# Gaukler/PlainRenderer

Hardware: AMD Instinct MI355X
Metric: frames/sec full GI+shade+post @4K; %HBM roofline; 1/2/4/8-GPU scaling (higher is better)
Workload: dtype f32

## Files before the change

### plainrenderer_amd/csrc/kernels_fast/shading_fast.hip

```cpp
#include "../backend.h"
#include "../device/shading_common.h"
#include "../device/fastmath.h"
#include "../device/buffer_fetch.h"
#include "upscale_quad.h"
#include "pcf_taps.h"
#include <type_traits>
#include <map>

namespace plr {

namespace fastshade {

#ifndef PLR_SHADE_WAVES
#define PLR_SHADE_WAVES 5
#endif

PLR_DI float rcpf(float x) { return __builtin_amdgcn_rcpf(x); }
PLR_DI float rsqf(float x) { return __builtin_amdgcn_rsqf(x); }
PLR_DI float sqrtv(float x) { return __builtin_amdgcn_sqrtf(x); }
PLR_DI float fmin1(float a, float b) { return __builtin_fminf(a, b); }
PLR_DI float fmax1(float a, float b) { return __builtin_fmaxf(a, b); }
PLR_DI float fclamp(float x, float lo, float hi) { return __builtin_fminf(__builtin_fmaxf(x, lo), hi); }
PLR_DI float fmix(float a, float b, float t) { return a + (b - a) * t; }
PLR_DI float log2h(float x) { return __builtin_amdgcn_logf(x); }
PLR_DI float exp2h(float x) { return __builtin_amdgcn_exp2f(x); }
PLR_DI vec3 nrm(vec3 v) { return v * rsqf(dot(v, v)); }
PLR_DI float pow5(float x) { x = fmax1(x, 0.f); const float x2 = x * x; return x2 * x2 * x; }
PLR_DI float fpow(float x, float y) { return x <= 0.f ? 0.f : exp2h(y * log2h(x)); }

PLR_DI float rcpRN(float d) { const float r = rcpf(d); return __builtin_fmaf(__builtin_fmaf(-d, r, 1.f), r, r); }
PLR_DI float divRNr(float n, float d, float r) { const float q = n * r; return __builtin_fmaf(__builtin_fmaf(-d, q, n), r, q); }
PLR_DI float divRN(float n, float d) { return divRNr(n, d, rcpf(d)); }
PLR_DI float sqrtRN(float x) { const float r = rsqf(x), s = x * r; return __builtin_fmaf(__builtin_fmaf(-s, s, x), 0.5f * r, s); }

struct ViewRay { vec3 Vn; float su, sv; };
PLR_DI ViewRay exactViewRay(const GlobalUbo* __restrict__ g, int px, int py) {
#pragma clang fp contract(off)
    ViewRay o;
// ... 91 lines not shown
    linearCoord(u * (float)im.w, &i0, &a);
    linearCoord(v * (float)im.h, &j0, &b);
    int xb; float a2;
    edgePair(i0, a, im.w, &xb, &a2);
    const int y0 = clampi(j0, im.h), y1 = clampi(j0 + 1, im.h);
    const BufferDesc texels = texelBuffer(im.ptr, 8u);
    const uint4 q0 = fetch128(texels, __umul24((uint32_t)y0, (uint32_t)im.w) + (uint32_t)xb), q1 = fetch128(texels, __umul24((uint32_t)y1, (uint32_t)im.w) + (uint32_t)xb);
    const float a0 = 1.f - a2, b0 = 1.f - b;
    vec4 r(0.f);
    r = accumulateTexel(r, q0.x, q0.y, a0 * b0);
    r = accumulateTexel(r, q0.z, q0.w, a2 * b0);
    r = accumulateTexel(r, q1.x, q1.y, a0 * b);
    r = accumulateTexel(r, q1.z, q1.w, a2 * b);
    return r;
}

struct ShadeParams {
    ImgView color, depth, normal, albedo, specular, brdfLut, shadowMaps[4], ysh, cocg, volumetricLut, skyLut;
    const LightBuffer* light;
    const ShadowCascadeInfo* shadowInfo;
    const VolumetricLightingSettings* vol;
    const GlobalUbo* g;
    const ImgView* bindless;
    uint32_t bindlessCount;
    uint32_t cascadeCount;
    int coverW, coverH, yBase;
    int xBase;
    uint32_t* sig;
    ImgView noiseTex;
    const float4* pcfTaps;
    const float4* pcfTapsByPosition;
    uint32_t pcfPositions;
    const uint2* lutEnergyFootprint;
};

#define PLR_SHADE_UNIFORM_PARAMS const GlobalUbo* __restrict__ gUniform, const LightBuffer* __restrict__ lightUniform, const ShadowCascadeInfo* __restrict__ shadowUniform, \
                                 const VolumetricLightingSettings* __restrict__ volUniform
#define PLR_SHADE_ADOPT_UNIFORMS(P) do { (P).g = gUniform; (P).light = lightUniform; (P).shadowInfo = shadowUniform; (P).vol = volUniform; } while (0)
#define PLR_SHADE_UNIFORM_ARGS(P) (P).g, (P).light, (P).shadowInfo, (P).vol

struct PcfTapRow { float4 q[kPcfTaps / 2]; };
PLR_DI float calcShadow(vec3 pos, const ImgView& shadowMap, const float* __restrict__ m, float lssX, float lssY, const PcfTapRow& taps) {
    float cxy0, cxy1;
    uint32_t depthThreshold;
    {
#pragma clang fp contract(off)
        const float x = ((m[0] * pos.x + m[4] * pos.y) + m[8] * pos.z) + m[12];
        const float y = ((m[1] * pos.x + m[5] * pos.y) + m[9] * pos.z) + m[13];
        const float z = ((m[2] * pos.x + m[6] * pos.y) + m[10] * pos.z) + m[14];
        const float w = ((m[3] * pos.x + m[7] * pos.y) + m[11] * pos.z) + m[15];
        const float rw = rcpf(w);
        cxy0 = divRNr(x, w, rw) * 0.5f + 0.5f;
        cxy1 = divRNr(y, w, rw) * 0.5f + 0.5f;
        const float actualDepth = fclamp(divRNr(z, w, rw), 0.f, 1.f);
        const uint32_t t0 = (uint32_t)(actualDepth * 65535.f);
        const float r16 = 1.f / 65535.f;
        const float q1 = divRNr((float)(t0 + 1u), 65535.f, r16), q0 = divRNr((float)t0, 65535.f, r16);
        depthThreshold = q1 <= actualDepth ? t0 + 1u : (q0 <= actualDepth ? t0 : t0 - 1u);
    }
    const int w = shadowMap.w, h = shadowMap.h;
    const float fw = (float)w, fh = (float)h;
    const float bxw = fastm::clampCoord(cxy0 * fw), byh = fastm::clampCoord(cxy1 * fh);
    const float sxw = 0.03f * lssX * fw, syh = 0.03f * lssY * fh;
    const __amdgpu_buffer_rsrc_t map = __builtin_amdgcn_make_buffer_rsrc(shadowMap.ptr, 0, w * h * 2, 0x00020000);
    uint32_t lit = 0u;
    auto tap = [&](float ox, float oy) {
        const int xi = floorToInt(__builtin_fmaf(ox, sxw, bxw)), yi = floorToInt(__builtin_fmaf(oy, syh, byh));
// ... 39 lines not shown
        const float unscaled = (1.f - energyIncoming) * (1.f - energyOutgoing) * rcpf(3.1415f * (1.f - energyAverage));
        const vec3 den = 1.f - fresnelAverage * (1.f - energyAverage);
        const vec3 scaling = (fresnelAverage * fresnelAverage * energyAverage) * vec3(rcpf(den.x), rcpf(den.y), rcpf(den.z));
        return unscaled * scaling;
    } else if (MULTISCATTER == 1) {
        const float lobe = (1.f - energyOutgoing) * (1.f / PLR_GLSL_PI);
        const vec3 den = 1.f - fresnelAverage * (1.f - energyOutgoing);
        return (fresnelAverage * fresnelAverage * (energyOutgoing * lobe)) * vec3(rcpf(den.x), rcpf(den.y), rcpf(den.z));
    } else if (MULTISCATTER == 2) {
        return f0 * (rcpf(energyOutgoing) - 1.f) * singleScatteringLobe;
    }
    return vec3(0.f);
}

struct PixelInputs {
    float depth;
    uint32_t albedo, specular;
    uint32_t normal, normalH, normalV;
    uint2 ysh;
    uint32_t cocg;
};
PLR_DI vec3 decodeNormal(uint32_t texel) {
    const vec3 raw = fastm::unorm8x4(texel).xyz() * 2.f - 1.f;
    return raw * rsqf(fmax1(dot(raw, raw), 1e-30f));
}

struct SurfaceTerms {
    vec3 N, V, f0, diffuseColor, diffuseBRDFIntegral;
    float r, NoV, energyOutgoing;
    vec3 brdfLut;
};
struct DirectOut { vec3 direct; float pixelDepth; vec2 noiseTexel; };
template <int DIFFUSE_BRDF, int MULTISCATTER, bool GEOMETRIC_AA>
PLR_DI DirectOut shadeDirect(const ShadeParams& P, int px, int py, const ViewRay& vr, const PixelInputs& in, vec3 lightColor, SurfaceTerms* st, uint32_t* sigWord) {
    const GlobalUbo* g = P.g;
    const Surface surf = exactSurface(g, vr.Vn, in.depth);
    const vec3 passPos = surf.passPos;
    const float pixelDepth = surf.pixelDepth;

    const vec3 albedoTexel = fastm::unorm8x4(in.albedo).xyz();
    const vec3 specularTexel = fastm::unorm8x4(in.specular).xyz();
    const float metalic = specularTexel.z;
    float r = specularTexel.y;
    r = fmax1(r * r, 0.0045f);
    const vec3 albedo(sRGBToLinear1(albedoTexel.x), sRGBToLinear1(albedoTexel.y), sRGBToLinear1(albedoTexel.z));
    const vec3 diffuseColor = (1.f - metalic) * albedo;
    const vec3 N = decodeNormal(in.normal);
    const vec3 L = nrm(ld3(g->sunDirection));
    const vec3 V = vr.Vn;
    const vec3 H = nrm(V + L);
    if (GEOMETRIC_AA) {
        const vec3 N_U = decodeNormal(in.normalH) - N, N_V = decodeNormal(in.normalV) - N;
        const float variance = 0.25f * (dot(N_V, N_V) + dot(N_U, N_U));
        const float kernelRoughness2 = fmin1(2.f * variance, 0.18f);
        r = fclamp(sqrtv(r * r + kernelRoughness2), 0.f, 1.f);
    }
    const float NoH = fmax1(dot(N, H), 0.f);
    const float NdotL = dot(N, L);
    const float NoL = fclamp(NdotL, 0.f, 1.f);
    const float VoH = fabsf(dot(V, H));
    const float LoV = fmax1(dot(L, V), 0.f);
    const float NoV = fmax1(fabsf(dot(N, V)), 0.0001f);
    const vec3 f0 = vmix(vec3(0.04f), albedo, metalic);

    const ImgView noiseTex = P.noiseTex;
    const uint32_t noiseIndex = fastm::texelIndex((uint32_t)fastm::repeatIndex(px, noiseTex.w), (uint32_t)fastm::repeatIndex(py, noiseTex.h), (uint32_t)noiseTex.w);
    const uint32_t noiseWord = fetch16(texelBuffer(noiseTex.ptr, 2u), noiseIndex);
    const vec2 noiseTexel = fastm::unorm8x2(noiseWord);
    const uint32_t noiseByte = noiseWord & 0xffu;

    int cascadeIndex = 0;
#pragma unroll
    for (int cascade = 0; cascade < 3; cascade++) cascadeIndex += (cascade < (int)P.cascadeCount - 1 && pixelDepth >= P.shadowInfo->splits[cascade]) ? 1 : 0;
    PcfTapRow tapRow;
    {
        const bool byPosition = P.pcfTapsByPosition != nullptr;
        const uint8_t* base = byPosition ? (const uint8_t*)P.pcfTapsByPosition : (const uint8_t*)P.pcfTaps;
        const uint32_t rowStride = byPosition ? P.pcfPositions * 16u : 16u;
        const uint32_t laneOffset = byPosition ? noiseIndex * 16u : noiseByte * (uint32_t)(kPcfTaps / 2 * 16);
        const __amdgpu_buffer_rsrc_t table = __builtin_amdgcn_make_buffer_rsrc((void*)base, 0, 0x7fffffff, 0x00020000);
#pragma unroll
        for (int k = 0; k < kPcfTaps / 2; k++) {
            const auto q = __builtin_amdgcn_raw_buffer_load_b128(table, (int)laneOffset, (int)((uint32_t)k * rowStride), 0);
            __builtin_memcpy(&tapRow.q[k], &q, 16);
        }
    }
    float sunShadow = 0.f;
    for (bool pending = true; pending;) {
        int c = __builtin_amdgcn_readfirstlane(cascadeIndex);
        const bool mine = cascadeIndex == c;
        asm volatile("" : "+s"(c));
        if (mine) {
            const ImgView& m0 = P.shadowMaps[0];
            ImgView shadowMap;
            shadowMap.ptr = c == 0 ? m0.ptr : c == 1 ? P.shadowMaps[1].ptr : c == 2 ? P.shadowMaps[2].ptr : P.shadowMaps[3].ptr;
            shadowMap.w = c == 0 ? m0.w : c == 1 ? P.shadowMaps[1].w : c == 2 ? P.shadowMaps[2].w : P.shadowMaps[3].w;
            shadowMap.h = c == 0 ? m0.h : c == 1 ? P.shadowMaps[1].h : c == 2 ? P.shadowMaps[2].h : P.shadowMaps[3].h;
            shadowMap.d = 1; shadowMap.fmt = F_D16;
            sunShadow = calcShadow(passPos, shadowMap, P.shadowInfo->lightMatrices[c], P.shadowInfo->lightSpaceScale[c][0], P.shadowInfo->lightSpaceScale[c][1], tapRow);
            pending = false;
        }
    }
    *sigWord = (uint32_t)cascadeIndex | ((uint32_t)(sunShadow * 12.f + 0.5f) << 2) | 64u;
    const vec3 directLighting = (fmax1(NdotL, 0.f) * sunShadow) * lightColor;
    const vec3 brdfLut = bilinearLut(P.brdfLut, r, NoV).xyz();

    vec3 diffuseDirect;
    vec3 diffuseBRDFIntegral(brdfLut.z);
    if (DIFFUSE_BRDF == 0) diffuseDirect = diffuseColor * (1.f / PLR_GLSL_PI) * directLighting;
    else if (DIFFUSE_BRDF == 1) diffuseDirect = DisneyDiffuse(diffuseColor, NoL, VoH, NoV, r) * directLighting;
    else if (DIFFUSE_BRDF == 2) diffuseDirect = CoDWWIIDiffuse(diffuseColor, NoL, VoH, NoV, NoH, r) * directLighting;
    else {
        const float single = Titanfall2DiffuseSingleComponent(NoL, LoV, NoV, NoH, r);
        diffuseDirect = diffuseColor * (single + diffuseColor * (0.1159f * r)) * directLighting;
        float multiIntegral = 0.1159f * r * PLR_GLSL_PI * 2.f;
        multiIntegral *= (1.f - (0.04f + 0.96f * pow5(1.f - NoV)));
        multiIntegral *= 0.94291f;
        diffuseBRDFIntegral = vmin(vec3(brdfLut.z) + diffuseColor * multiIntegral, vec3(1.f));
    }
    diffuseDirect = diffuseDirect * ((1.f - F_Schlick(f0, vec3(1.f), NoV)) * (1.f - F_Schlick(f0, vec3(1.f), NoL)));

    const vec3 singleScatteringLobe = GGXSingleScattering(r, f0, NoH, NoV, VoH, NoL);
    const vec3 multiScatteringLobe = specularMultiscatteringLobe<MULTISCATTER>(P, r, NoL, f0, singleScatteringLobe, brdfLut);
    const vec3 specularDirect = directLighting * (singleScatteringLobe + multiScatteringLobe);

    st->N = N; st->V = V; st->f0 = f0; st->diffuseColor = diffuseColor; st->diffuseBRDFIntegral = diffuseBRDFIntegral;
    st->r = r; st->NoV = NoV; st->energyOutgoing = brdfLut.y; st->brdfLut = brdfLut;
    DirectOut o;
    o.direct = diffuseDirect + specularDirect;
    o.pixelDepth = pixelDepth;
    o.noiseTexel = noiseTexel;
    return o;
}

template <int MULTISCATTER>
PLR_DI vec3 shadeIndirect(const ShadeParams& P, const SurfaceTerms& st, uint2 ysh, uint32_t cocg) {
    const vec3 N = st.N, V = st.V, f0 = st.f0;
    const float r = st.r, NoV = st.NoV;
    const vec4 irradiance_Y_SH(halfBitsToFloat(ysh.x & 0xffffu), halfBitsToFloat(ysh.x >> 16), halfBitsToFloat(ysh.y & 0xffffu), halfBitsToFloat(ysh.y >> 16));
    const vec2 cc(halfBitsToFloat(cocg & 0xffffu), halfBitsToFloat(cocg >> 16));
    const vec4 shN(0.5f, -0.8660254f * N.y, 0.8660254f * N.z, -0.8660254f * N.x);
    const float irradiance_Y = dot(irradiance_Y_SH, shN);
    const vec3 irradiance = YCoCgToLinear(vec3(irradiance_Y, cc.x, cc.y));
    const vec3 diffuseIndirect = irradiance * st.diffuseColor * st.diffuseBRDFIntegral;
    const vec3 dominantDirection = dominantDirectionFromSH_L1(irradiance_Y_SH);
    const float dominantDirectionLength = fclamp(sqrtv(dot(dominantDirection, dominantDirection)), 0.01f, 1.f);
    const float r_indirect = fmix(1.f, r, sqrtv(dominantDirectionLength));
    const vec3 L_indirect = dominantDirection * rcpf(dominantDirectionLength);
    const vec3 H_indirect = nrm(L_indirect + V);
    const float NoH_indirect = fmax1(dot(N, H_indirect), 0.f);
    const float NoL_indirect = fmax1(dot(N, L_indirect), 0.f);
    const float VoH_indirect = fmax1(dot(V, H_indirect), 0.f);
    const vec3 single_i = GGXSingleScattering(r_indirect, f0, NoH_indirect, NoV, VoH_indirect, NoL_indirect);
    const vec3 multi_i = specularMultiscatteringLobe<MULTISCATTER>(P, r_indirect, NoL_indirect, f0, single_i, vec3(0.f, st.energyOutgoing, 0.f));
    const vec3 specularIndirect = (single_i + multi_i) * YCoCgToLinear(vec3(irradiance_Y_SH.x, cc.x, cc.y));
    return diffuseIndirect + specularIndirect;
}

PLR_DI vec4 froxelLookup(const ShadeParams& P, float su, float sv, vec2 noiseTexel, float pixelDepth) {
    const float nu = su + (noiseTexel.x - 0.5f) * 0.013f, nv = sv + (noiseTexel.y - 0.5f) * 0.013f;
    const float linear = pixelDepth * rcpf(P.vol->maxDistance);
    const float z = log2h(linear * 19.0855369f + 1.f) * (0.693147181f / 3.f);
    const ImgView& vol = P.volumetricLut;
    int i0, j0, k0; float a, b, c;
    linearCoord(nu * (float)vol.w, &i0, &a);
    linearCoord(nv * (float)vol.h, &j0, &b);
    linearCoord(z * (float)vol.d, &k0, &c);
    int xb; float a2;
    edgePair(i0, a, vol.w, &xb, &a2);
    const uint32_t y0 = __umul24((uint32_t)clampi(j0, vol.h), (uint32_t)vol.w), y1 = __umul24((uint32_t)clampi(j0 + 1, vol.h), (uint32_t)vol.w);
    const uint32_t sl = (uint32_t)vol.w * (uint32_t)vol.h;
    const uint32_t z0 = __umul24((uint32_t)clampi(k0, vol.d), sl), z1 = __umul24((uint32_t)clampi(k0 + 1, vol.d), sl);
    const BufferDesc texels = texelBuffer(vol.ptr, 8u);
    const uint32_t x0 = (uint32_t)xb;
    const uint4 q00 = fetch128(texels, z0 + y0 + x0), q01 = fetch128(texels, z0 + y1 + x0), q10 = fetch128(texels, z1 + y0 + x0), q11 = fetch128(texels, z1 + y1 + x0);
    const float a0 = 1.f - a2, b0 = 1.f - b, c0 = 1.f - c;
    const float wab00 = a0 * b0, wab10 = a2 * b0, wab01 = a0 * b, wab11 = a2 * b;
    vec4 it(0.f);
    it = accumulateTexel(it, q00.x, q00.y, wab00 * c0);
    it = accumulateTexel(it, q00.z, q00.w, wab10 * c0);
    it = accumulateTexel(it, q01.x, q01.y, wab01 * c0);
    it = accumulateTexel(it, q01.z, q01.w, wab11 * c0);
    it = accumulateTexel(it, q10.x, q10.y, wab00 * c);
    it = accumulateTexel(it, q10.z, q10.w, wab10 * c);
    it = accumulateTexel(it, q11.x, q11.y, wab01 * c);
    it = accumulateTexel(it, q11.z, q11.w, wab11 * c);
    return it;
}

template <int DIFFUSE_BRDF, int MULTISCATTER, bool GEOMETRIC_AA, int INDIRECT_TECH>
PLR_DI uint32_t shadeGeometryPixel(const ShadeParams& P, int px, int py, const ViewRay& vr, const PixelInputs& in, uint32_t* sigWord) {
    SurfaceTerms st;
    const DirectOut d = shadeDirect<DIFFUSE_BRDF, MULTISCATTER, GEOMETRIC_AA>(P, px, py, vr, in, ld3(P.light->sunColor), &st, sigWord);
    vec3 lightingIndirect;
    if (INDIRECT_TECH == 0) lightingIndirect = shadeIndirect<MULTISCATTER>(P, st, in.ysh, in.cocg);
    else {
        const float amb = 0.003f * P.light->sunStrengthExposed;
        const vec3 singleScattering = vmix(vec3(st.brdfLut.x), vec3(st.brdfLut.y), st.f0);
        lightingIndirect = (amb * st.diffuseColor) * st.diffuseBRDFIntegral + singleScattering * amb;
    }
    vec3 outColor = d.direct * P.light->sunStrengthExposed + lightingIndirect;
    const vec4 it = froxelLookup(P, vr.su, vr.sv, d.noiseTexel, d.pixelDepth);
    outColor = outColor * it.w + it.xyz();
    return packR11G11B10(outColor);
}

template <int DIFFUSE_BRDF, int MULTISCATTER, bool GEOMETRIC_AA, int INDIRECT_TECH>
__global__ __launch_bounds__(256, PLR_SHADE_WAVES) void deferredShadingFastKernel(ShadeParams P, PLR_SHADE_UNIFORM_PARAMS) {
    PLR_SHADE_ADOPT_UNIFORMS(P);
    const int px = P.xBase + (int)(blockIdx.x * 64u + (threadIdx.x & 63u));
    const int py = P.yBase + (int)(blockIdx.y * 4u + (threadIdx.x >> 6));
    if (px >= P.coverW || py >= P.coverH) return;
    const ViewRay vr = exactViewRay(P.g, px, py);
    const uint32_t idx = fastm::texelIndex((uint32_t)px, (uint32_t)py, (uint32_t)P.color.w);
    PixelInputs in;
    in.depth = ((const float*)P.depth.ptr)[idx];
    if (in.depth == 0.f) {
        ((uint32_t*)P.color.ptr)[idx] = packR11G11B10(fastm::sampleSkyLut(-vr.Vn, P.skyLut));
        if (P.sig) P.sig[idx] = 128u;
        return;
    }
    in.albedo = ((const uint32_t*)P.albedo.ptr)[idx];
    in.specular = ((const uint32_t*)P.specular.ptr)[idx];
    const uint32_t* normals = (const uint32_t*)P.normal.ptr;
    const uint32_t nw = (uint32_t)P.normal.w;
    const int nx = clampi(px, P.normal.w), ny = clampi(py, P.normal.h);
// ... 113 lines not shown
    if (P.sig) P.sig[idx] = sigWord | (upSig << 8);
}

struct DirectRecords { uint4* a; uint4* b; uint32_t* c; };
PLR_DI uint32_t packHalves(float lo, float hi) { return __builtin_bit_cast(uint32_t, __builtin_amdgcn_cvt_pkrtz(lo, hi)); }

template <int DIFFUSE_BRDF, int MULTISCATTER, bool GEOMETRIC_AA>
__global__ __launch_bounds__(256, PLR_SHADE_WAVES) void shadeDirectKernel(ShadeParams P, DirectRecords R, const GlobalUbo G, const ShadowCascadeInfo* __restrict__ shadowUniform,
                                                                          const VolumetricLightingSettings* __restrict__ volUniform) {
    P.g = &G; P.shadowInfo = shadowUniform; P.vol = volUniform; P.light = nullptr;
    const int px = P.xBase + (int)(blockIdx.x * 64u + (threadIdx.x & 63u));
    const int py = P.yBase + (int)(blockIdx.y * 4u + (threadIdx.x >> 6));
    if (px >= P.coverW || py >= P.coverH) return;
    const ViewRay vr = exactViewRay(P.g, px, py);
    const uint32_t idx = fastm::texelIndex((uint32_t)px, (uint32_t)py, (uint32_t)P.color.w);
    PixelInputs in;
    in.depth = u2f(fetch32(texelBuffer(P.depth.ptr, 4u), idx));
    if (in.depth == 0.f) {
        R.a[idx] = make_uint4(packR11G11B10(fastm::sampleSkyLut(-vr.Vn, P.skyLut)), 0u, 0u, 0u);
        return;
    }
    in.albedo = fetch32(texelBuffer(P.albedo.ptr, 4u), idx);
    in.specular = fetch32(texelBuffer(P.specular.ptr, 4u), idx);
    in.normal = fetch32(texelBuffer(P.normal.ptr, 4u), idx);
    in.normalH = in.normalV = in.normal;
    if (GEOMETRIC_AA) {
        in.normalH = fetch32(texelBuffer(P.normal.ptr, 4u), fastm::texelIndex((uint32_t)clampi(px ^ 1, P.normal.w), (uint32_t)py, (uint32_t)P.normal.w));
        in.normalV = fetch32(texelBuffer(P.normal.ptr, 4u), fastm::texelIndex((uint32_t)px, (uint32_t)clampi(py ^ 1, P.normal.h), (uint32_t)P.normal.w));
    }
    in.ysh = make_uint2(0u, 0u);
    in.cocg = 0u;
    SurfaceTerms st;
    uint32_t sigWord;
    const DirectOut d = shadeDirect<DIFFUSE_BRDF, MULTISCATTER, GEOMETRIC_AA>(P, px, py, vr, in, vec3(1.f), &st, &sigWord);
    const vec4 it = froxelLookup(P, vr.su, vr.sv, d.noiseTexel, d.pixelDepth);
    const vec3 X = d.direct * it.w;
    const vec3 dci = st.diffuseColor * st.diffuseBRDFIntegral;
    R.a[idx] = make_uint4(f2u(X.x), f2u(X.y), f2u(X.z), packHalves(it.w, st.r));
    R.b[idx] = make_uint4(packHalves(it.x, it.y), packHalves(it.z, st.energyOutgoing), packHalves(dci.x, dci.y), packHalves(dci.z, st.f0.x));
    R.c[idx] = packHalves(st.f0.y, st.f0.z);
}

template <int MULTISCATTER>
__global__ __launch_bounds__(256) void upscaleAndCombineKernel(ShadeParams P, FusedUpscale U, DirectRecords R, const GlobalUbo* __restrict__ gUniform, const LightBuffer* __restrict__ lightUniform) {
    P.g = gUniform; P.light = lightUniform;
    __shared__ GiTexel tile[kGiTileH][kGiTileW];
    const int t = (int)threadIdx.x;
    const int X0 = P.xBase + (int)(blockIdx.x * 64u), Y0 = P.yBase + (int)(blockIdx.y * 4u);
    const int k0 = (X0 >> 1) - 1, m0 = (Y0 >> 1) - 1;
    const GlobalUbo* g = P.g;
    const float nearP = g->nearPlane, farP = g->farPlane, nf = nearP * farP, nmf = nearP - farP;
    if (t < kGiTileW * kGiTileH) {
        const int r = t / kGiTileW, c = t - r * kGiTileW;
        const int hw = U.srcYSH.w, hh = U.srcYSH.h;
        const uint32_t i = fastm::texelIndex((uint32_t)clampi(k0 + c, hw), (uint32_t)clampi(m0 + r, hh), (uint32_t)hw);
        const uint2 ys = fetch64(texelBuffer(U.srcYSH.ptr, 8u), i);
        const uint32_t cc = fetch32(texelBuffer(U.srcCoCg.ptr, 4u), i);
        GiTexel e;
        e.depthLinear = fastquad::linearDepthRounded(halfBitsToFloat(fetch16(texelBuffer(U.halfResDepth.ptr, 2u), i)), nf, nmf, farP);
        e.y0 = halfBitsToFloat(ys.x & 0xffffu); e.y1 = halfBitsToFloat(ys.x >> 16); e.y2 = halfBitsToFloat(ys.y & 0xffffu); e.y3 = halfBitsToFloat(ys.y >> 16);
        e.co = halfBitsToFloat(cc & 0xffffu); e.cg = halfBitsToFloat(cc >> 16); e.pad = 0.f;
        tile[r][c] = e;
    }
    const int px = X0 + (t & 63), py = Y0 + (t >> 6);
    const bool covered = px < P.coverW && py < P.coverH;
    const int cpx = covered ? px : 0, cpy = covered ? py : 0;
    const uint32_t idx = fastm::texelIndex((uint32_t)cpx, (uint32_t)cpy, (uint32_t)P.color.w);
// ... 67 lines not shown
    const vec3 inScattering((float)halfLo(rb.x), (float)halfHi(rb.x), (float)halfLo(rb.y));
    const vec3 light = ld3(P.light->sunColor) * P.light->sunStrengthExposed;
    const vec3 outColor = vec3(u2f(ra.x), u2f(ra.y), u2f(ra.z)) * light + (lightingIndirect * transmittance + inScattering);
    ((uint32_t*)P.color.ptr)[idx] = packR11G11B10(outColor);
}

typedef void (*ShadeKernel)(ShadeParams, const GlobalUbo*, const LightBuffer*, const ShadowCascadeInfo*, const VolumetricLightingSettings*);
template <int D, int M, bool G> static ShadeKernel pickIndirect(int tech) {
    return tech == 0 ? (ShadeKernel)deferredShadingFastKernel<D, M, G, 0> : (ShadeKernel)deferredShadingFastKernel<D, M, G, 1>;
}
template <int D, int M> static ShadeKernel pickAA(bool aa, int tech) { return aa ? pickIndirect<D, M, true>(tech) : pickIndirect<D, M, false>(tech); }
template <int D> static ShadeKernel pickMulti(int m, bool aa, int tech) {
    switch (m) {
        case 0: return pickAA<D, 0>(aa, tech);
        case 1: return pickAA<D, 1>(aa, tech);
        case 2: return pickAA<D, 2>(aa, tech);
        default: return pickAA<D, 3>(aa, tech);
    }
}
typedef void (*FusedKernel)(ShadeParams, FusedUpscale, const GlobalUbo*, const LightBuffer*, const ShadowCascadeInfo*, const VolumetricLightingSettings*);
template <int D, int M> static FusedKernel pickFusedAA(bool aa) { return aa ? (FusedKernel)upscaleAndShadeKernel<D, M, true> : (FusedKernel)upscaleAndShadeKernel<D, M, false>; }
template <int D> static FusedKernel pickFusedMulti(int m, bool aa) {
    switch (m) {
        case 0: return pickFusedAA<D, 0>(aa);
        case 1: return pickFusedAA<D, 1>(aa);
        case 2: return pickFusedAA<D, 2>(aa);
        default: return pickFusedAA<D, 3>(aa);
    }
}

constexpr int kNoiseSlots = 4;
constexpr uint32_t kMaxNoisePositions = 4096;
constexpr size_t kNoiseSlotBytes = (size_t)kMaxNoisePositions * (kPcfTaps / 2) * sizeof(float4);
__global__ void lutEnergyFootprintKernel(ImgView lut, uint2* __restrict__ out) {
    const int x = (int)(blockIdx.x * 64u + (threadIdx.x & 63u)), y = (int)(blockIdx.y * 4u + (threadIdx.x >> 6));
    if (x >= lut.w - 1 || y >= lut.h - 1) return;
    const uint2* t = (const uint2*)lut.ptr;
    auto energy = [&](int tx, int ty) { return t[(size_t)ty * (size_t)lut.w + tx].x >> 16; };
    out[(size_t)y * (size_t)(lut.w - 1) + x] = make_uint2(energy(x, y) | (energy(x + 1, y) << 16), energy(x, y + 1) | (energy(x + 1, y + 1) << 16));
}
__global__ void pcfTapsByPositionKernel(const uint16_t* __restrict__ noiseTexels, uint32_t positions, const float4* __restrict__ byValue, float4* __restrict__ byPosition) {
    const uint32_t pos = blockIdx.x * blockDim.x + threadIdx.x;
    if (pos >= positions) return;
    const uint32_t noiseByte = noiseTexels[pos] & 0xffu;
    const float2* taps = (const float2*)byValue + noiseByte * kPcfTaps;
    const int turn = (int)((float)noiseByte * (12.f / 255.f) + 0.5f);
#pragma unroll
    for (int k = 0; k < kPcfTaps / 2; k++) {
        const int i0 = ((2 * k - turn) % kPcfTaps + kPcfTaps) % kPcfTaps, i1 = ((2 * k + 1 - turn) % kPcfTaps + kPcfTaps) % kPcfTaps;
        byPosition[(uint32_t)k * positions + pos] = make_float4(taps[i0].x, taps[i0].y, taps[i1].x, taps[i1].y);
    }
}
struct ShadeDerived {
    const void* scratchBase = nullptr;
    size_t scratchBytes = 0;
    struct Slot { const void* noise = nullptr; int w = 0, h = 0; uint64_t version = 0, lastUse = 0; } slots[kNoiseSlots];
    uint64_t useCounter = 0;
    const void* lut = nullptr; int lutW = 0, lutH = 0; uint64_t lutVersion = 0;
};
static thread_local std::map<const void*, ShadeDerived> g_shadeDerived;
static int shadeDerivedTables(const PassCtx& c, ShadeParams* P, DirectRecords* records = nullptr) {
    const ImgView& lut = P->brdfLut;
    const size_t footprintOffset = kPcfTapTableBytes + kNoiseSlots * kNoiseSlotBytes;
    const size_t footprintBytes = (size_t)(lut.w - 1) * (size_t)std::max(lut.h - 1, 1) * sizeof(uint2);
    const size_t recordsOffset = (footprintOffset + footprintBytes + 255) & ~(size_t)255;
    const size_t pixels = (size_t)P->color.w * (size_t)P->color.h;
    const size_t total = records ? recordsOffset + pixels * 36 : footprintOffset + footprintBytes;
    uint8_t* scratch = (uint8_t*)c.scratch(total);
    if (!scratch) return c.fail(-2, "deferredShading: cannot allocate scratch memory");
    if (records) { records->a = (uint4*)(scratch + recordsOffset); records->b = records->a + pixels; records->c = (uint32_t*)(records->b + pixels); }
    ShadeDerived& d = g_shadeDerived[(const void*)c.scratchSlot];
    if (d.scratchBase != scratch || d.scratchBytes != *c.scratchSize) {
        d = ShadeDerived{};
        d.scratchBase = scratch;
        d.scratchBytes = *c.scratchSize;
        const hipError_t e = buildPcfTapTable((float2*)scratch, c.stream);
        if (e != hipSuccess) return c.fail(-2, std::string("deferredShading: PCF tap table: ") + hipGetErrorString(e));
    }
    P->pcfTaps = (const float4*)scratch;
    P->pcfTapsByPosition = nullptr;
    P->pcfPositions = 0;
    P->lutEnergyFootprint = nullptr;
    if (const uint64_t lutVersion = lut.h >= 2 ? contentVersionOf(lut.ptr) : 0) {
        if (d.lut != lut.ptr || d.lutW != lut.w || d.lutH != lut.h || d.lutVersion != lutVersion) {
            lutEnergyFootprintKernel<<<dim3(divUp((unsigned)(lut.w - 1), 64u), divUp((unsigned)(lut.h - 1), 4u)), 256, 0, c.stream>>>(lut, (uint2*)(scratch + footprintOffset));
            PLR_CHECK_LAUNCH(c);
            d.lut = lut.ptr; d.lutW = lut.w; d.lutH = lut.h; d.lutVersion = lutVersion;
        }
        P->lutEnergyFootprint = (const uint2*)(scratch + footprintOffset);
    }
    const ImgView& noise = P->noiseTex;
    if (!noise.ptr || noise.fmt != F_RG8) return 0;
    const uint64_t version = contentVersionOf(noise.ptr);
    const uint64_t positions = (uint64_t)noise.w * (uint64_t)noise.h;
    if (version == 0 || positions > kMaxNoisePositions) return 0;
    ShadeDerived::Slot* slot = nullptr;
    for (auto& s : d.slots) if (s.noise == noise.ptr && s.w == noise.w && s.h == noise.h && s.version == version) slot = &s;
    if (!slot) {
        slot = &d.slots[0];
        for (auto& s : d.slots) if (s.lastUse < slot->lastUse) slot = &s;
        float4* dst = (float4*)(scratch + kPcfTapTableBytes + (size_t)(slot - d.slots) * kNoiseSlotBytes);
        pcfTapsByPositionKernel<<<divUp((unsigned)positions, 256u), 256, 0, c.stream>>>((const uint16_t*)noise.ptr, (uint32_t)positions, (const float4*)scratch, dst);
        PLR_CHECK_LAUNCH(c);
        slot->noise = noise.ptr; slot->w = noise.w; slot->h = noise.h; slot->version = version;
    }
    slot->lastUse = ++d.useCounter;
    P->pcfTapsByPosition = (const float4*)(scratch + kPcfTapTableBytes + (size_t)(slot - d.slots) * kNoiseSlotBytes);
    P->pcfPositions = (uint32_t)positions;
    return 0;
}

static int shadeParamsFor(const PassCtx& c, ShadeParams* out, int* diffuseBRDF, int* multi, bool* aa, int* tech, bool deriveTables = true, DirectRecords* records = nullptr) {
    if (int rc = c.needGlobal()) return rc;
    if (int rc = c.needStorage(0, F_R11G11B10, "deferredShading colour target")) return rc;
    if (int rc = c.needSampled(3, F_RGBA16F, "deferredShading brdfLutTexture")) return rc;
    if (int rc = c.needSbuf(7, sizeof(LightBuffer), "deferredShading lightBuffer")) return rc;
    if (int rc = c.needSbuf(8, sizeof(ShadowCascadeInfo), "deferredShading sunShadowInfo")) return rc;
    for (int i = 0; i < 4; i++) if (int rc = c.needSampled(9 + i, F_D16, "deferredShading shadowMapCascade")) return rc;
    if (int rc = c.needSampled(15, F_RGBA16F, "deferredShading indirectDiffuse_Y_SH")) return rc;
    if (int rc = c.needSampled(16, F_RG16F, "deferredShading indirectDiffuse_CoCg")) return rc;
    if (int rc = c.needSampled(18, F_RGBA16F, "deferredShading volumetricLightingLUT")) return rc;
    if (int rc = c.needUbuf(19, 52, "deferredShading volumetric settings")) return rc;
    if (int rc = c.needSampled(20, F_D32, "deferredShading depth")) return rc;
    if (int rc = c.needSampled(21, F_RGBA8, "deferredShading world normals")) return rc;
    if (int rc = c.needSampled(22, F_RGBA8, "deferredShading albedo")) return rc;
    if (int rc = c.needSampled(23, F_RGBA8, "deferredShading specular")) return rc;
    if (int rc = c.needSampled(24, F_R11G11B10, "deferredShading skyLut")) return rc;
    if (!c.bindless || c.bindlessCount == 0) return c.fail(-4, "deferredShading: global texture array (set 2) is empty");
    if (c.sampled[16].w != c.sampled[15].w || c.sampled[16].h != c.sampled[15].h) return c.fail(-4, "deferredShading: Y_SH and CoCg differ in size");
    for (int b : {20, 22, 23}) if (c.sampled[b].w != c.storage[0].w || c.sampled[b].h != c.storage[0].h) return kUseGeneralKernel;
    if (c.sampled[3].w < 2 || c.sampled[18].w < 2) return kUseGeneralKernel;
    *diffuseBRDF = c.specInt(0, 0); *multi = c.specInt(1, 0); *tech = c.specInt(3, 0);
    *aa = c.specBool(2, false);
    const uint32_t cascades = c.specUint(4, 4u);
    if (*diffuseBRDF < 0 || *diffuseBRDF > 3 || *multi < 0 || *multi > 3 || cascades < 1 || cascades > 4) return c.fail(-1, "deferredShading: specialisation constant out of range");
    ShadeParams P{};
    P.color = c.storage[0]; P.depth = c.sampled[20]; P.normal = c.sampled[21]; P.albedo = c.sampled[22]; P.specular = c.sampled[23];
    P.brdfLut = c.sampled[3];
    for (int i = 0; i < 4; i++) P.shadowMaps[i] = c.sampled[9 + i];
    P.ysh = c.sampled[15]; P.cocg = c.sampled[16]; P.volumetricLut = c.sampled[18]; P.skyLut = c.sampled[24];
    P.light = (const LightBuffer*)c.sbuf[7].ptr; P.shadowInfo = (const ShadowCascadeInfo*)c.sbuf[8].ptr;
    P.vol = (const VolumetricLightingSettings*)c.ubuf[19].ptr; P.g = c.global;
    P.bindless = c.bindless; P.bindlessCount = c.bindlessCount; P.cascadeCount = cascades;
    if (!c.hostNoiseView(&P.noiseTex)) return kUseGeneralKernel;
    if (deriveTables) if (int rc = shadeDerivedTables(c, &P, records)) return rc;
    const PassCtx::RowSpan rs = c.rowSpan(P.color.h);
    const PassCtx::ColSpan cs = c.colSpan(P.color.w);
    P.coverW = cs.x1; P.xBase = cs.x0; P.coverH = rs.y1; P.yBase = rs.y0;
    P.sig = c.sigFor((size_t)P.color.w * (size_t)P.color.h);
    *out = P;
    return 0;
}

static int launchDeferredShadingFast(const PassCtx& c) {
    ShadeParams P;
    int diffuseBRDF, multi, tech;
    bool aa;
    if (int rc = shadeParamsFor(c, &P, &diffuseBRDF, &multi, &aa, &tech)) return rc;
    ShadeKernel k = nullptr;
    switch (diffuseBRDF) {
        case 0: k = pickMulti<0>(multi, aa, tech); break;
        case 1: k = pickMulti<1>(multi, aa, tech); break;
        case 2: k = pickMulti<2>(multi, aa, tech); break;
        default: k = pickMulti<3>(multi, aa, tech); break;
    }
    if (P.coverW <= P.xBase || P.coverH <= P.yBase) return 0;
    k<<<dim3(divUp((unsigned)(P.coverW - P.xBase), 64u), divUp((unsigned)(P.coverH - P.yBase), 4u)), 256, 0, c.stream>>>(P, PLR_SHADE_UNIFORM_ARGS(P));
    PLR_CHECK_LAUNCH(c);
    return 0;
}

struct FusedShade { ShadeParams P; FusedUpscale U; int diffuseBRDF, multi; bool aa; };
static int fusedShadeSetup(const PassCtx* const* ctxs, size_t count, FusedShade* f, bool deriveTables, DirectRecords* records) {
    if (count != 2) return kUseGeneralKernel;
    const PassCtx &u = *ctxs[0], &c = *ctxs[1];
    if (!u.global || !u.hasStorage(0) || !u.hasStorage(1) || !u.hasSampled(2) || !u.hasSampled(3) || !u.hasSampled(4) || !u.hasSampled(5)) return kUseGeneralKernel;
    if (u.storage[0].fmt != F_RGBA16F || u.storage[1].fmt != F_RG16F || u.sampled[2].fmt != F_RGBA16F || u.sampled[3].fmt != F_RG16F || u.sampled[4].fmt != F_D32 ||
        u.sampled[5].fmt != F_R16F)
        return kUseGeneralKernel;
    const ImgView& out = u.storage[0];
    const PassCtx::RowSpan ur = u.rowSpan(out.h);
    const bool regular = out.w == 2 * u.sampled[2].w && out.h == 2 * u.sampled[2].h && u.sampled[3].w == u.sampled[2].w && u.sampled[3].h == u.sampled[2].h &&
// ... 194 lines not shown
```

Measured before the change: 1427.

## Skip shadow PCF and BRDF lobe evaluation for back-facing or fully shadowed pixels

Adds an unlit fast path to deferred shading. Shadow-map PCF sampling is skipped for back-facing pixels, and the diffuse and specular lobes are skipped when the pixel is back-facing or fully shadowed. Safety guards check finiteness of the sun colour and LUT energy, with a flag set by the footprint kernel. The path is disabled when signature output is requested or an environment variable turns it off, so it trades extra uniform checks and branching for less ALU and memory work on unlit pixels.

```diff
diff --git a/plainrenderer_amd/csrc/kernels_fast/shading_fast.hip b/plainrenderer_amd/csrc/kernels_fast/shading_fast.hip
--- a/plainrenderer_amd/csrc/kernels_fast/shading_fast.hip
+++ b/plainrenderer_amd/csrc/kernels_fast/shading_fast.hip
@@ -4,6 +4,7 @@
 #include "../device/buffer_fetch.h"
 #include "upscale_quad.h"
 #include "pcf_taps.h"
+#include <cstdlib>
 #include <type_traits>
 #include <map>
 
@@ -161,7 +162,11 @@
     const float4* pcfTapsByPosition;
     uint32_t pcfPositions;
     const uint2* lutEnergyFootprint;
+    const uint32_t* lutEnergyNonFinite;
+    uint32_t skipUnlit;
 };
+PLR_DI float uniformValue(float x) { return u2f((uint32_t)__builtin_amdgcn_readfirstlane((int)f2u(x))); }
+PLR_DI bool finiteBits(float x) { return (f2u(x) & 0x7f800000u) != 0x7f800000u; }
 
 #define PLR_SHADE_UNIFORM_PARAMS const GlobalUbo* __restrict__ gUniform, const LightBuffer* __restrict__ lightUniform, const ShadowCascadeInfo* __restrict__ shadowUniform, \
                                  const VolumetricLightingSettings* __restrict__ volUniform
@@ -267,7 +272,11 @@
 };
 struct DirectOut { vec3 direct; float pixelDepth; vec2 noiseTexel; };
 template <int DIFFUSE_BRDF, int MULTISCATTER, bool GEOMETRIC_AA>
-PLR_DI DirectOut shadeDirect(const ShadeParams& P, int px, int py, const ViewRay& vr, const PixelInputs& in, vec3 lightColor, SurfaceTerms* st, uint32_t* sigWord) {
+PLR_DI DirectOut shadeDirect(const ShadeParams& P, bool skipUnlit, int px, int py, const ViewRay& vr, const PixelInputs& in, vec3 lightColor, SurfaceTerms* st,
+                             uint32_t* sigWord) {
+    constexpr bool kLobesSkippable = DIFFUSE_BRDF != 3 && (MULTISCATTER == 0 || MULTISCATTER == 3);
+    uint32_t lutNonFinite = 1u;
+    if (kLobesSkippable && MULTISCATTER == 0 && skipUnlit && P.lutEnergyNonFinite) lutNonFinite = *P.lutEnergyNonFinite;
     const GlobalUbo* g = P.g;
     const Surface surf = exactSurface(g, vr.Vn, in.depth);
     const vec3 passPos = surf.passPos;
@@ -282,19 +291,17 @@
     const vec3 diffuseColor = (1.f - metalic) * albedo;
     const vec3 N = decodeNormal(in.normal);
     const vec3 L = nrm(ld3(g->sunDirection));
+    const vec3 Lu(uniformValue(L.x), uniformValue(L.y), uniformValue(L.z));
     const vec3 V = vr.Vn;
-    const vec3 H = nrm(V + L);
     if (GEOMETRIC_AA) {
         const vec3 N_U = decodeNormal(in.normalH) - N, N_V = decodeNormal(in.normalV) - N;
         const float variance = 0.25f * (dot(N_V, N_V) + dot(N_U, N_U));
         const float kernelRoughness2 = fmin1(2.f * variance, 0.18f);
         r = fclamp(sqrtv(r * r + kernelRoughness2), 0.f, 1.f);
     }
-    const float NoH = fmax1(dot(N, H), 0.f);
     const float NdotL = dot(N, L);
     const float NoL = fclamp(NdotL, 0.f, 1.f);
-    const float VoH = fabsf(dot(V, H));
-    const float LoV = fmax1(dot(L, V), 0.f);
+    const bool backFacing = NdotL <= 0.f;
     const float NoV = fmax1(fabsf(dot(N, V)), 0.0001f);
     const vec3 f0 = vmix(vec3(0.04f), albedo, metalic);
 
@@ -307,62 +314,76 @@
     int cascadeIndex = 0;
 #pragma unroll
     for (int cascade = 0; cascade < 3; cascade++) cascadeIndex += (cascade < (int)P.cascadeCount - 1 && pixelDepth >= P.shadowInfo->splits[cascade]) ? 1 : 0;
-    PcfTapRow tapRow;
-    {
-        const bool byPosition = P.pcfTapsByPosition != nullptr;
-        const uint8_t* base = byPosition ? (const uint8_t*)P.pcfTapsByPosition : (const uint8_t*)P.pcfTaps;
-        const uint32_t rowStride = byPosition ? P.pcfPositions * 16u : 16u;
-        const uint32_t laneOffset = byPosition ? noiseIndex * 16u : noiseByte * (uint32_t)(kPcfTaps / 2 * 16);
-        const __amdgpu_buffer_rsrc_t table = __builtin_amdgcn_make_buffer_rsrc((void*)base, 0, 0x7fffffff, 0x00020000);
+    const bool skipLobes = kLobesSkippable && skipUnlit && (MULTISCATTER != 0 || __builtin_amdgcn_readfirstlane(lutNonFinite) == 0u);
+    float sunShadow = 0.f;
+    if (!(skipUnlit && backFacing)) {
+        PcfTapRow tapRow;
+        {
+            const bool byPosition = P.pcfTapsByPosition != nullptr;
+            const uint8_t* base = byPosition ? (const uint8_t*)P.pcfTapsByPosition : (const uint8_t*)P.pcfTaps;
+            const uint32_t rowStride = byPosition ? P.pcfPositions * 16u : 16u;
+            const uint32_t laneOffset = byPosition ? noiseIndex * 16u : noiseByte * (uint32_t)(kPcfTaps / 2 * 16);
+            const __amdgpu_buffer_rsrc_t table = __builtin_amdgcn_make_buffer_rsrc((void*)base, 0, 0x7fffffff, 0x00020000);
 #pragma unroll
-        for (int k = 0; k < kPcfTaps / 2; k++) {
-            const auto q = __builtin_amdgcn_raw_buffer_load_b128(table, (int)laneOffset, (int)((uint32_t)k * rowStride), 0);
-            __builtin_memcpy(&tapRow.q[k], &q, 16);
+            for (int k = 0; k < kPcfTaps / 2; k++) {
+                const auto q = __builtin_amdgcn_raw_buffer_load_b128(table, (int)laneOffset, (int)((uint32_t)k * rowStride), 0);
+                __builtin_memcpy(&tapRow.q[k], &q, 16);
+            }
         }
-    }
-    float sunShadow = 0.f;
-    for (bool pending = true; pending;) {
-        int c = __builtin_amdgcn_readfirstlane(cascadeIndex);
-        const bool mine = cascadeIndex == c;
-        asm volatile("" : "+s"(c));
-        if (mine) {
-            const ImgView& m0 = P.shadowMaps[0];
-            ImgView shadowMap;
-            shadowMap.ptr = c == 0 ? m0.ptr : c == 1 ? P.shadowMaps[1].ptr : c == 2 ? P.shadowMaps[2].ptr : P.shadowMaps[3].ptr;
-            shadowMap.w = c == 0 ? m0.w : c == 1 ? P.shadowMaps[1].w : c == 2 ? P.shadowMaps[2].w : P.shadowMaps[3].w;
-            shadowMap.h = c == 0 ? m0.h : c == 1 ? P.shadowMaps[1].h : c == 2 ? P.shadowMaps[2].h : P.shadowMaps[3].h;
-            shadowMap.d = 1; shadowMap.fmt = F_D16;
-            sunShadow = calcShadow(passPos, shadowMap, P.shadowInfo->lightMatrices[c], P.shadowInfo->lightSpaceScale[c][0], P.shadowInfo->lightSpaceScale[c][1], tapRow);
-            pending = false;
+        for (bool pending = true; pending;) {
+            int c = __builtin_amdgcn_readfirstlane(cascadeIndex);
+            const bool mine = cascadeIndex == c;
+            asm volatile("" : "+s"(c));
+            if (mine) {
+                const ImgView& m0 = P.shadowMaps[0];
+                ImgView shadowMap;
+                shadowMap.ptr = c == 0 ? m0.ptr : c == 1 ? P.shadowMaps[1].ptr : c == 2 ? P.shadowMaps[2].ptr : P.shadowMaps[3].ptr;
+                shadowMap.w = c == 0 ? m0.w : c == 1 ? P.shadowMaps[1].w : c == 2 ? P.shadowMaps[2].w : P.shadowMaps[3].w;
+                shadowMap.h = c == 0 ? m0.h : c == 1 ? P.shadowMaps[1].h : c == 2 ? P.shadowMaps[2].h : P.shadowMaps[3].h;
+                shadowMap.d = 1; shadowMap.fmt = F_D16;
+                sunShadow = calcShadow(passPos, shadowMap, P.shadowInfo->lightMatrices[c], P.shadowInfo->lightSpaceScale[c][0], P.shadowInfo->lightSpaceScale[c][1], tapRow);
+                pending = false;
+            }
         }
     }
     *sigWord = (uint32_t)cascadeIndex | ((uint32_t)(sunShadow * 12.f + 0.5f) << 2) | 64u;
-    const vec3 directLighting = (fmax1(NdotL, 0.f) * sunShadow) * lightColor;
     const vec3 brdfLut = bilinearLut(P.brdfLut, r, NoV).xyz();
 
-    vec3 diffuseDirect;
+    const vec3 VL = V + Lu;
+    const float VL2 = dot(VL, VL);
+    const bool unlit = skipLobes && (backFacing || sunShadow == 0.f) && VL2 >= 1e-30f && VL2 <= 8.f;
+    vec3 direct(0.f);
     vec3 diffuseBRDFIntegral(brdfLut.z);
-    if (DIFFUSE_BRDF == 0) diffuseDirect = diffuseColor * (1.f / PLR_GLSL_PI) * directLighting;
-    else if (DIFFUSE_BRDF == 1) diffuseDirect = DisneyDiffuse(diffuseColor, NoL, VoH, NoV, r) * directLighting;
-    else if (DIFFUSE_BRDF == 2) diffuseDirect = CoDWWIIDiffuse(diffuseColor, NoL, VoH, NoV, NoH, r) * directLighting;
-    else {
-        const float single = Titanfall2DiffuseSingleComponent(NoL, LoV, NoV, NoH, r);
-        diffuseDirect = diffuseColor * (single + diffuseColor * (0.1159f * r)) * directLighting;
-        float multiIntegral = 0.1159f * r * PLR_GLSL_PI * 2.f;
-        multiIntegral *= (1.f - (0.04f + 0.96f * pow5(1.f - NoV)));
-        multiIntegral *= 0.94291f;
-        diffuseBRDFIntegral = vmin(vec3(brdfLut.z) + diffuseColor * multiIntegral, vec3(1.f));
-    }
-    diffuseDirect = diffuseDirect * ((1.f - F_Schlick(f0, vec3(1.f), NoV)) * (1.f - F_Schlick(f0, vec3(1.f), NoL)));
-
-    const vec3 singleScatteringLobe = GGXSingleScattering(r, f0, NoH, NoV, VoH, NoL);
-    const vec3 multiScatteringLobe = specularMultiscatteringLobe<MULTISCATTER>(P, r, NoL, f0, singleScatteringLobe, brdfLut);
-    const vec3 specularDirect = directLighting * (singleScatteringLobe + multiScatteringLobe);
+    if (!unlit) {
+        const vec3 H = VL * rsqf(VL2);
+        const float NoH = fmax1(dot(N, H), 0.f);
+        const float VoH = fabsf(dot(V, H));
+        const float LoV = fmax1(dot(Lu, V), 0.f);
+        const vec3 directLighting = (fmax1(NdotL, 0.f) * sunShadow) * lightColor;
+        vec3 diffuseDirect;
+        if (DIFFUSE_BRDF == 0) diffuseDirect = diffuseColor * (1.f / PLR_GLSL_PI) * directLighting;
+        else if (DIFFUSE_BRDF == 1) diffuseDirect = DisneyDiffuse(diffuseColor, NoL, VoH, NoV, r) * directLighting;
+        else if (DIFFUSE_BRDF == 2) diffuseDirect = CoDWWIIDiffuse(diffuseColor, NoL, VoH, NoV, NoH, r) * directLighting;
+        else {
+            const float single = Titanfall2DiffuseSingleComponent(NoL, LoV, NoV, NoH, r);
+            diffuseDirect = diffuseColor * (single + diffuseColor * (0.1159f * r)) * directLighting;
+            float multiIntegral = 0.1159f * r * PLR_GLSL_PI * 2.f;
+            multiIntegral *= (1.f - (0.04f + 0.96f * pow5(1.f - NoV)));
+            multiIntegral *= 0.94291f;
+            diffuseBRDFIntegral = vmin(vec3(brdfLut.z) + diffuseColor * multiIntegral, vec3(1.f));
+        }
+        diffuseDirect = diffuseDirect * ((1.f - F_Schlick(f0, vec3(1.f), NoV)) * (1.f - F_Schlick(f0, vec3(1.f), NoL)));
+
+        const vec3 singleScatteringLobe = GGXSingleScattering(r, f0, NoH, NoV, VoH, NoL);
+        const vec3 multiScatteringLobe = specularMultiscatteringLobe<MULTISCATTER>(P, r, NoL, f0, singleScatteringLobe, brdfLut);
+        const vec3 specularDirect = directLighting * (singleScatteringLobe + multiScatteringLobe);
+        direct = diffuseDirect + specularDirect;
+    }
 
     st->N = N; st->V = V; st->f0 = f0; st->diffuseColor = diffuseColor; st->diffuseBRDFIntegral = diffuseBRDFIntegral;
     st->r = r; st->NoV = NoV; st->energyOutgoing = brdfLut.y; st->brdfLut = brdfLut;
     DirectOut o;
-    o.direct = diffuseDirect + specularDirect;
+    o.direct = direct;
     o.pixelDepth = pixelDepth;
     o.noiseTexel = noiseTexel;
     return o;
@@ -426,7 +447,9 @@
 template <int DIFFUSE_BRDF, int MULTISCATTER, bool GEOMETRIC_AA, int INDIRECT_TECH>
 PLR_DI uint32_t shadeGeometryPixel(const ShadeParams& P, int px, int py, const ViewRay& vr, const PixelInputs& in, uint32_t* sigWord) {
     SurfaceTerms st;
-    const DirectOut d = shadeDirect<DIFFUSE_BRDF, MULTISCATTER, GEOMETRIC_AA>(P, px, py, vr, in, ld3(P.light->sunColor), &st, sigWord);
+    const vec3 sunColor = ld3(P.light->sunColor);
+    const bool skipUnlit = P.skipUnlit && finiteBits(sunColor.x) && finiteBits(sunColor.y) && finiteBits(sunColor.z) && finiteBits(P.light->sunStrengthExposed);
+    const DirectOut d = shadeDirect<DIFFUSE_BRDF, MULTISCATTER, GEOMETRIC_AA>(P, skipUnlit, px, py, vr, in, sunColor, &st, sigWord);
     vec3 lightingIndirect;
     if (INDIRECT_TECH == 0) lightingIndirect = shadeIndirect<MULTISCATTER>(P, st, in.ysh, in.cocg);
     else {
@@ -606,7 +629,7 @@
     in.cocg = 0u;
     SurfaceTerms st;
     uint32_t sigWord;
-    const DirectOut d = shadeDirect<DIFFUSE_BRDF, MULTISCATTER, GEOMETRIC_AA>(P, px, py, vr, in, vec3(1.f), &st, &sigWord);
+    const DirectOut d = shadeDirect<DIFFUSE_BRDF, MULTISCATTER, GEOMETRIC_AA>(P, P.skipUnlit != 0u, px, py, vr, in, vec3(1.f), &st, &sigWord);
     const vec4 it = froxelLookup(P, vr.su, vr.sv, d.noiseTexel, d.pixelDepth);
     const vec3 X = d.direct * it.w;
     const vec3 dci = st.diffuseColor * st.diffuseBRDFIntegral;
@@ -740,12 +763,15 @@
 constexpr int kNoiseSlots = 4;
 constexpr uint32_t kMaxNoisePositions = 4096;
 constexpr size_t kNoiseSlotBytes = (size_t)kMaxNoisePositions * (kPcfTaps / 2) * sizeof(float4);
-__global__ void lutEnergyFootprintKernel(ImgView lut, uint2* __restrict__ out) {
+__global__ void lutEnergyFootprintKernel(ImgView lut, uint2* __restrict__ out, uint32_t* __restrict__ nonFinite) {
     const int x = (int)(blockIdx.x * 64u + (threadIdx.x & 63u)), y = (int)(blockIdx.y * 4u + (threadIdx.x >> 6));
     if (x >= lut.w - 1 || y >= lut.h - 1) return;
     const uint2* t = (const uint2*)lut.ptr;
     auto energy = [&](int tx, int ty) { return t[(size_t)ty * (size_t)lut.w + tx].x >> 16; };
-    out[(size_t)y * (size_t)(lut.w - 1) + x] = make_uint2(energy(x, y) | (energy(x + 1, y) << 16), energy(x, y + 1) | (energy(x + 1, y + 1) << 16));
+    const uint32_t e00 = energy(x, y), e10 = energy(x + 1, y), e01 = energy(x, y + 1), e11 = energy(x + 1, y + 1);
+    out[(size_t)y * (size_t)(lut.w - 1) + x] = make_uint2(e00 | (e10 << 16), e01 | (e11 << 16));
+    auto special = [](uint32_t h) { return (h & 0x7c00u) == 0x7c00u; };
+    if (special(e00) || special(e10) || special(e01) || special(e11)) *nonFinite = 1u;
 }
 __global__ void pcfTapsByPositionKernel(const uint16_t* __restrict__ noiseTexels, uint32_t positions, const float4* __restrict__ byValue, float4* __restrict__ byPosition) {
     const uint32_t pos = blockIdx.x * blockDim.x + threadIdx.x;
@@ -771,9 +797,10 @@
     const ImgView& lut = P->brdfLut;
     const size_t footprintOffset = kPcfTapTableBytes + kNoiseSlots * kNoiseSlotBytes;
     const size_t footprintBytes = (size_t)(lut.w - 1) * (size_t)std::max(lut.h - 1, 1) * sizeof(uint2);
-    const size_t recordsOffset = (footprintOffset + footprintBytes + 255) & ~(size_t)255;
+    const size_t flagOffset = (footprintOffset + footprintBytes + 15) & ~(size_t)15;
+    const size_t recordsOffset = (flagOffset + 16 + 255) & ~(size_t)255;
     const size_t pixels = (size_t)P->color.w * (size_t)P->color.h;
-    const size_t total = records ? recordsOffset + pixels * 36 : footprintOffset + footprintBytes;
+    const size_t total = records ? recordsOffset + pixels * 36 : flagOffset + 16;
     uint8_t* scratch = (uint8_t*)c.scratch(total);
     if (!scratch) return c.fail(-2, "deferredShading: cannot allocate scratch memory");
     if (records) { records->a = (uint4*)(scratch + recordsOffset); records->b = records->a + pixels; records->c = (uint32_t*)(records->b + pixels); }
@@ -789,13 +816,18 @@
     P->pcfTapsByPosition = nullptr;
     P->pcfPositions = 0;
     P->lutEnergyFootprint = nullptr;
+    P->lutEnergyNonFinite = nullptr;
     if (const uint64_t lutVersion = lut.h >= 2 ? contentVersionOf(lut.ptr) : 0) {
         if (d.lut != lut.ptr || d.lutW != lut.w || d.lutH != lut.h || d.lutVersion != lutVersion) {
-            lutEnergyFootprintKernel<<<dim3(divUp((unsigned)(lut.w - 1), 64u), divUp((unsigned)(lut.h - 1), 4u)), 256, 0, c.stream>>>(lut, (uint2*)(scratch + footprintOffset));
+            const hipError_t e = hipMemsetAsync(scratch + flagOffset, 0, 16, c.stream);
+            if (e != hipSuccess) return c.fail(-2, std::string("deferredShading: LUT energy footprint: ") + hipGetErrorString(e));
+            lutEnergyFootprintKernel<<<dim3(divUp((unsigned)(lut.w - 1), 64u), divUp((unsigned)(lut.h - 1), 4u)), 256, 0, c.stream>>>(lut, (uint2*)(scratch + footprintOffset),
+                                                                                                                                       (uint32_t*)(scratch + flagOffset));
             PLR_CHECK_LAUNCH(c);
             d.lut = lut.ptr; d.lutW = lut.w; d.lutH = lut.h; d.lutVersion = lutVersion;
         }
         P->lutEnergyFootprint = (const uint2*)(scratch + footprintOffset);
+        P->lutEnergyNonFinite = (const uint32_t*)(scratch + flagOffset);
     }
     const ImgView& noise = P->noiseTex;
     if (!noise.ptr || noise.fmt != F_RG8) return 0;
@@ -856,6 +888,8 @@
     const PassCtx::ColSpan cs = c.colSpan(P.color.w);
     P.coverW = cs.x1; P.xBase = cs.x0; P.coverH = rs.y1; P.yBase = rs.y0;
     P.sig = c.sigFor((size_t)P.color.w * (size_t)P.color.h);
+    const char* skipEnv = std::getenv("PLR_SHADE_SKIP_UNLIT");
+    P.skipUnlit = (!P.sig && !(skipEnv && skipEnv[0] == '0' && skipEnv[1] == 0)) ? 1u : 0u;
     *out = P;
     return 0;
 }
```

Result: faster. 1471, median of 6 (+3.0%).
